# jordanshivers/optical-flow-python

Hardware: AMD Instinct MI355X
Metric: image-pairs/sec at 1920x1080 Classic+NL-fast (+ ms/pyramid-level, AEPE) (higher is better)
Workload: dtype f32; 1 GPU; classic+nl-fast on synth_pair(1080,1920,seed) RGB, 8 pair(s)/GPU/step, 4 in flight; method=classic+nl-fast, height=1080, width=1920, pairs_per_gpu=8, lanes=4, solver=backslash (GPU block-Jacobi PCG surrogate), parallelism=pairs sharded 1/GPU x 1, RCCL gather

## Files before the change

### include/optflow.h

```cpp
#ifndef OPTFLOW_H
#define OPTFLOW_H

#include <stdint.h>

#ifdef __cplusplus
extern "C" {
#endif

#define OF_ABI_VERSION 3

#define OF_OK 0
#define OF_EINVAL (-1)
#define OF_EHIP (-2)
#define OF_ENOMEM (-3)
#define OF_ENOTSUP (-4)
#define OF_ERCCL (-5)

enum of_method { OF_METHOD_HS = 0, OF_METHOD_BA = 1, OF_METHOD_CLASSIC_NL = 2, OF_METHOD_ALT_BA = 3 };

enum of_interp { OF_INTERP_CUBIC = 0 ,
                 OF_INTERP_BICUBIC = 1 ,
                 OF_INTERP_BILINEAR = 2  };

enum of_solver { OF_SOLVER_BACKSLASH = 0, OF_SOLVER_PCG = 1, OF_SOLVER_SOR = 2 };
// ... 83 lines not shown
  double total_ms;
  double preprocess_ms;
} of_stats;

typedef struct of_ctx of_ctx;

int of_abi_version(void);
int of_device_count(int *count);
int of_ctx_create(int device, of_ctx **out);
int of_ctx_destroy(of_ctx *ctx);
const char *of_last_error(of_ctx *ctx);
int of_synchronize(of_ctx *ctx);
int of_set_profiling(of_ctx *ctx, int enable);
#define OF_OPT_SOR_PIPELINE 1
#define OF_OPT_FUSED_WARP 3
int of_set_option(of_ctx *ctx, int option, int value);
#define OF_OPT_SOR_FALLBACKS 2
#define OF_OPT_DEVICE_BYTES 4
#define OF_OPT_RCCL_NRANKS 5
int of_get_option(of_ctx *ctx, int option, int64_t *value);
enum of_event { OF_EV_STAGE = 0, OF_EV_LEVEL = 1, OF_EV_ITER = 2, OF_EV_STAGE_END = 3 };
#define OF_PROGRESS_ITER 1
#define OF_PROGRESS_FLOW 2
typedef struct of_progress {
  int32_t event;
  int32_t stage;
  int32_t level;
  int32_t h, w;
  int32_t iter, lin;
  int32_t pad_;
// ... 103 lines not shown
```

### optical-flow-python_amd/csrc/api.hip

```cpp
extern "C" {

int of_abi_version(void) { return OF_ABI_VERSION; }

int of_device_count(int *count) {
  int n = 0;
  if (hipGetDeviceCount(&n) != hipSuccess) n = 0;
  if (count) *count = n;
  return OF_OK;
}

int of_ctx_create(int device, of_ctx **out) {
  if (!out) return OF_EINVAL;
  *out = nullptr;
  int n = 0;
  if (hipGetDeviceCount(&n) != hipSuccess || device < 0 || device >= n) {
    g_err = "no HIP device";
    return OF_EHIP;
  }
  of_ctx *c = new of_ctx();
  c->device = device;
  try {
    HIPCHK(hipSetDevice(device));
    create_stream(&c->stream);
    HIPCHK(hipMalloc(&c->d_state, sizeof(PcgState)));
// ... 77 lines not shown
  if ((c)->pool) {                                                                   \
    (c)->err = "a pair stream is open on this context (of_pairs_close first)";       \
    return OF_EINVAL;                                                                \
  }

int of_set_option(of_ctx *c, int option, int value) {
  if (!c) return OF_EINVAL;
  REFUSE_WHILE_POOL(c)
  switch (option) {
    case OF_OPT_SOR_PIPELINE:
      c->opt_sor_pipe = value < 0 ? 0 : (value > 2 ? 2 : value);
      return OF_OK;
    case OF_OPT_FUSED_WARP:
      c->opt_fused_warp = value ? 1 : 0;
      return OF_OK;
    default:
      c->err = "unknown option";
      return OF_EINVAL;
  }
}

int of_set_progress(of_ctx *c, of_progress_fn fn, void *user, int flags) {
  if (!c) return OF_EINVAL;
  if (c->pool) pool_set_progress(c->pool, fn);
  else c->prog_fn = fn;
  c->prog_user = user;
  c->prog_flags = flags;
  return OF_OK;
}

int of_get_option(of_ctx *c, int option, int64_t *value) {
  if (!c || !value) return OF_EINVAL;
  switch (option) {
    case OF_OPT_SOR_PIPELINE:
      *value = c->opt_sor_pipe;
      return OF_OK;
    case OF_OPT_FUSED_WARP:
      *value = c->opt_fused_warp;
      return OF_OK;
    case OF_OPT_SOR_FALLBACKS: {
      int64_t n = c->sor_fallbacks;
      for (of_ctx *l : c->lanes) n += l->sor_fallbacks;
      *value = n;
      return OF_OK;
    }
    case OF_OPT_DEVICE_BYTES: {
      auto held = [](const of_ctx *x) {
        return (int64_t)(x->arena.reserved() + x->sor_ring_cap + x->gather_cap);
      };
      int64_t n = held(c);
      for (of_ctx *l : c->lanes) n += held(l);
      *value = n;
      return OF_OK;
// ... 367 lines not shown
  download_f2(c, xx, x);
  HIPCHK(hipStreamSynchronize(c->stream));
  if (iters) *iters = r.iters;
  if (rel_residual) *rel_residual = r.rel;
  API_END(c)
}
int of_detect_occlusion(of_ctx *c, const float *uv, const float *images, int H, int W, int nc, float *occ) {
  API_BEGIN(c)
  REQUIRE(uv && images && occ && nc >= 1, OF_EINVAL, "bad arguments");
  F2 f = upload_f2(c, uv, H, W), z = new_f2(c, H, W), u1 = new_f2(c, H, W);
  fill_f2(c, z, 0.0f);
  Img im = upload_new_img(c, images, H, W, 2 * nc);
  Img o = new_img(c, H, W, 1);
  Grid2 g = grid2(H, W);
  launch(c, "update_occ", k_update_occ, g.grid, g.block, 0, (const float2 *)f.p, (const float2 *)z.p, 0, u1.p,
         (const float *)im.p, (const float *)im.plane(nc), nc, o.p, H, W, f.P, im.ps());
  download_img(c, o, occ);
  HIPCHK(hipStreamSynchronize(c->stream));
  API_END(c)
}

int of_weighted_median(of_ctx *c, const float *uv, const float *guide, int gc, const float *occ, int H, int W,
                       int area_hsz, double sigma_i, float *out) {
  API_BEGIN(c)
  REQUIRE(uv && guide && occ && out && gc >= 1, OF_EINVAL, "bad arguments");
  F2 f = upload_f2(c, uv, H, W), o = new_f2(c, H, W);
  Img g = upload_new_img(c, guide, H, W, gc), oc = upload_new_img(c, occ, H, W, 1);
  wmf(c, f, g, oc.p, o, area_hsz, sigma_i);
  download_f2(c, o, out);
  HIPCHK(hipStreamSynchronize(c->stream));
  API_END(c)
// ... 78 lines not shown
```

### optical-flow-python_amd/csrc/batch.hip

```cpp
namespace {

void ensure_lanes(of_ctx *c, int n) {
  const int want = std::max(n, OF_LANES_MIN - 1);
  while ((int)c->lanes.size() < want) {
    of_ctx *l = nullptr;
    const int rc = of_ctx_create(c->device, &l);
    REQUIRE(rc == OF_OK, rc, "lane context: " + g_err);
    c->lanes.push_back(l);
  }
  if (!c->gstream) create_stream(&c->gstream);
}

of_ctx *lane_ctx(of_ctx *c, int li) { return li ? c->lanes[li - 1] : c; }

void configure_lane(of_ctx *parent, of_ctx *lane, int prof, bool token_on) {
  if (lane != parent) {
    lane->prof = prof;
    lane->epoch = parent->epoch;
  }
  lane->opt_sor_pipe = parent->opt_sor_pipe;
  lane->opt_fused_warp = parent->opt_fused_warp;
  lane->big = token_on && OF_BIG_PX > 0 ? &parent->big_own : nullptr;
  lane->big_px = OF_BIG_PX;
}

void merge_lane_prof(of_ctx *c, int lanes) {
  c->big = nullptr;
  for (int li = 1; li < lanes; ++li) {
    of_ctx *l = c->lanes[li - 1];
    for (auto &kv : l->ktimes) {
      KTime &d = c->ktimes[kv.first];
      d.ms += kv.second.ms;
      d.px += kv.second.px;
      d.n += kv.second.n;
    }
    l->ktimes.clear();
    c->tl.insert(c->tl.end(), l->tl.begin(), l->tl.end());
    l->tl.clear();
// ... 661 lines not shown
```

### optical-flow-python_amd/csrc/host_core.h

```cpp
namespace {

struct OfError {
  int code;
  std::string msg;
};

#define HIPCHK(x)                                                                                    \
  do {                                                                                               \
    hipError_t e_ = (x);                                                                             \
    if (e_ != hipSuccess) throw OfError{OF_EHIP, std::string(#x) + ": " + hipGetErrorString(e_)}; \
  } while (0)
#define REQUIRE(cond, code, msg) \
  do {                           \
    if (!(cond)) throw OfError{code, msg}; \
  } while (0)

#ifndef OF_TOKEN_SLOTS
#define OF_TOKEN_SLOTS 2
#endif
struct Token {
  std::mutex m;
  std::condition_variable cv;
  int free = OF_TOKEN_SLOTS;
  void lock() {
// ... 49 lines not shown
    size_t n = 0;
    for (const auto &c : chunks) n += c.cap;
    return n;
  }
};

struct Img {
  float *p = nullptr;
  int H = 0, W = 0, P = 0, C = 0;
  size_t ps() const { return (size_t)H * P; }
  float *plane(int c) const { return p + (size_t)c * ps(); }
};
struct F2 {
  float2 *p = nullptr;
  int H = 0, W = 0, P = 0;
};

struct ProfRec {
  const char *name;
  hipEvent_t e0, e1;
  double px;
};
struct KTime {
  double ms = 0, px = 0;
  int64_t n = 0;
};

struct Slot {
  void *rgb1 = nullptr, *rgb2 = nullptr;
  float *uv = nullptr;
// ... 123 lines not shown
    const char *name;
    double px, t0, t1;
  };
  std::vector<TlRec> tl;
  hipEvent_t epoch = nullptr;
  bool own_epoch = false;
  std::map<int64_t, int> iter_hints;
  double cur_px = 0;
  std::vector<Slot> slots;
  HostStage *hs = nullptr;
  PairPool *pool = nullptr;
  std::vector<of_ctx *> lanes;
  Token big_own;
  Token *big = nullptr;
  double big_px = 0;
  ncclComm_t comm = nullptr;
  int nranks = 1, rank = 0;
};

namespace {

hipEvent_t next_event(std::vector<hipEvent_t> &pool, size_t &used) {
  if (used == pool.size()) {
    hipEvent_t e;
    HIPCHK(hipEventCreate(&e));
    pool.push_back(e);
  }
  return pool[used++];
}
hipEvent_t pool_event(of_ctx *c) { return next_event(c->ev_pool, c->ev_used); }
// ... 92 lines not shown
```

### optical-flow-python_amd/csrc/host_flow.hip

```cpp
namespace {

OpArgs op_args(const of_params *P, double alpha, double lambda2) {
  OpArgs o;
  memset(&o, 0, sizeof(o));
  o.qd = to_penf(P->qua_data);
  o.rd = to_penf(P->rho_data);
  for (int k = 0; k < 2; ++k) {
    o.qsu[k] = to_penf(P->qua_spatial_u[k]);
    o.qsv[k] = to_penf(P->qua_spatial_v[k]);
    o.rsu[k] = to_penf(P->rho_spatial_u[k]);
    o.rsv[k] = to_penf(P->rho_spatial_v[k]);
  }
  o.rc = to_penf(P->rho_couple);
  o.use_q = alpha > 0.0;
  o.use_r = alpha < 1.0;
  o.aq_s = (float)((o.use_r ? alpha : 1.0) * P->lambda_q);
  o.ar_s = (float)((o.use_q ? 1.0 - alpha : 1.0) * P->lambda_);
  o.aq_d = (float)(o.use_r ? alpha : 1.0);
  o.ar_d = (float)(o.use_q ? 1.0 - alpha : 1.0);
  o.lambda2 = (float)lambda2;
  o.f64 = P->method == OF_METHOD_ALT_BA;
  o.aq_s_d = (o.use_r ? alpha : 1.0) * P->lambda_q;
  o.ar_s_d = (o.use_q ? 1.0 - alpha : 1.0) * P->lambda_;
  o.aq_d_d = o.use_r ? alpha : 1.0;
// ... 67 lines not shown
    if (one) { OF_BY_PM(m, k_warp_operator, 2, 1, ) } else { OF_BY_PM(m, k_warp_operator, 2, 3, ) }
  }
}

struct LevelIn {
  Img im;
  Img guide;
};

struct BigPhase {
  of_ctx *c;
  bool held = false;
  BigPhase(of_ctx *c_, double px) : c(c_) {
    if (c->big && px >= c->big_px) {
      c->big->lock();
      held = true;
    }
  }
  ~BigPhase() {
    if (held) {
      hipStreamSynchronize(c->stream);
      c->big->unlock();
    }
  }
};

SolveResult solve_tok(of_ctx *c, const of_params *P, const Img &coef, const F2 &b, const F2 &x) {
  BigPhase bp(c, (double)b.H * b.W);
  return solve(c, P, coef, b, x);
}

struct ProgressOff {
  of_ctx *c;
  of_progress_fn fn;
  explicit ProgressOff(of_ctx *c_) : c(c_), fn(c_->prog_fn) { c->prog_fn = nullptr; }
  ~ProgressOff() { c->prog_fn = fn; }
// ... 70 lines not shown
  c->cur_px = (double)H * W;
  const double blend = P->method == OF_METHOD_BA ? P->blend : 0.5;
  LevelDeriv D = level_deriv(c, L.im, nc, P->interp, P->deriv_filter, blend);
  Img It = new_img(c, H, W, nc), Ix = new_img(c, H, W, nc), Iy = new_img(c, H, W, nc);
  Img coef = new_img(c, H, W, 7);
  Img occ = new_img(c, H, W, 1);
  F2 rhs = new_f2(c, H, W), x = new_f2(c, H, W), uv1 = new_f2(c, H, W), uv2 = new_f2(c, H, W);
  F2 duv = new_f2(c, H, W);
  OpArgs o = op_args(P, alpha, 0.0);
  Grid2 g = grid2(H, W);
  const bool nl = P->method == OF_METHOD_CLASSIC_NL;
  const bool gen = P->filters.general;
  GenLevel GL;
  if (gen) GL = gen_level(c, P, H, W);
  const bool fuse = !gen && max_linear == 1 && can_fuse_warp_op(c, o, nc);
  for (int it = 0; it < P->max_iters; ++it) {
    if (!fuse) partial_deriv(c, D, P->interp, uv, It, Ix, Iy);
    for (int jl = 0; jl < max_linear; ++jl) {
      if (gen) {
        gen_flow_operator(c, P, o, uv, jl ? &duv : nullptr, It, Ix, Iy, nullptr, GL, rhs);
        note_solve(c, st, gen_solve_logged(c, P, GL, rhs, x));
      } else if (fuse) {
        warp_operator(c, D, P->interp, o, uv, coef, rhs);
        note_solve(c, st, solve_tok(c, P, coef, rhs, x));
      } else {
        flow_operator(c, o, uv, jl ? &duv : nullptr, It, Ix, Iy, nullptr, coef, rhs);
        note_solve(c, st, solve_tok(c, P, coef, rhs, x));
      }
      c->cur_px = (double)H * W;
      prog_iter(c, it, jl, x, jl ? &duv : nullptr, P->limit_update);
      const bool filt = P->median_filter_size != 0;
      launch(c, nl && filt && L.guide.p ? "update_occ" : "update", k_update_occ, g.grid, g.block, 0,
             (const float2 *)uv.p, (const float2 *)x.p, P->limit_update, uv1.p, (const float *)L.im.p,
             (const float *)L.im.plane(nc), nc, (nl && filt && L.guide.p) ? occ.p : (float *)nullptr, H, W, uv.P,
             L.im.ps());
      const bool last = jl + 1 >= max_linear;
      if (last && filt && nl && L.guide.p) {
        wmf(c, uv1, L.guide, occ.p, uv, P->area_hsz, P->sigma_i, (const float2 *)uv.p);
        continue;
      }
      F2 res = uv1;
      if (filt) {
        if (nl && L.guide.p) wmf(c, uv1, L.guide, occ.p, uv2, P->area_hsz, P->sigma_i);
        else median2(c, uv1, uv2, P->median_filter_size);
        res = uv2;
      }
      if (!last)
        launch(c, "sub2", k_sub2, g.grid, g.block, 0, (const float2 *)uv.p, (const float2 *)res.p, duv.p, H, W, uv.P);
      else
        launch(c, "axpy_diff", k_axpy_diff, g.grid, g.block, 0, uv.p, (const float2 *)uv.p, (const float2 *)res.p, H,
// ... 120 lines not shown
    levels = auto_levels(H, W, P->pyramid_spacing);
  P->pyramid_levels = levels;
  REQUIRE(levels <= OF_MAX_LEVELS, OF_EINVAL, "too many pyramid levels");
  FlowPyr F;
  F.levels = levels;
  F.pyr = build_pyramid(c, img, levels, P->pyramid_spacing);
  if (P->method != OF_METHOD_HS) F.gpyr = build_pyramid(c, img, P->gnc_pyramid_levels, P->gnc_pyramid_spacing);
  guide_pyramids(c, P, guide, F);
  return F;
}

void run_schedule(of_ctx *c, of_params *P, const FlowPyr &F, F2 &uv_io, of_stats *st) {
  const int H = uv_io.H, W = uv_io.W, levels = F.levels;
  const std::vector<Img> &pyr = F.pyr, &gpyr = F.gpyr, &cpyr = F.cpyr, &cgpyr = F.cgpyr;
  const bool use_guide = F.use_guide;
  F2 uv = uv_io, uvhat;
  if (P->method == OF_METHOD_ALT_BA) {
    uvhat = new_f2(c, H, W);
    HIPCHK(hipMemcpyAsync(uvhat.p, uv.p, sizeof(float2) * (size_t)H * uv.P, hipMemcpyDeviceToDevice, c->stream));
  }
  const double alpha_orig = P->alpha;
  const int gnc = P->method == OF_METHOD_HS ? 1 : P->gnc_iters;
  std::vector<std::pair<hipEvent_t, hipEvent_t>> lev_ev;
  for (int ig = 0; ig < gnc; ++ig) {
    const int nl = ig == 0 ? levels : P->gnc_pyramid_levels;
    const std::vector<Img> &lv = ig == 0 ? pyr : gpyr;
    c->prog_stage = ig;
    c->prog_level = -1;
    if (c->prog_fn) {
      of_progress e = prog_event(c, OF_EV_STAGE, H, W);
// ... 192 lines not shown
```

### optical-flow-python_amd/csrc/host_image.hip

```cpp
namespace {

Img new_img(of_ctx *c, int H, int W, int C) {
  Img m;
  m.H = H;
  m.W = W;
  m.C = C;
  m.P = of_pitch(W);
  m.p = (float *)c->arena.alloc(sizeof(float) * m.ps() * (C > 0 ? C : 1));
  return m;
}
F2 new_f2(of_ctx *c, int H, int W) {
  F2 f;
  f.H = H;
  f.W = W;
  f.P = of_pitch(W);
  f.p = (float2 *)c->arena.alloc(sizeof(float2) * (size_t)H * f.P);
  return f;
}
Img view(const Img &m, int c0, int n) {
  Img v = m;
  v.p = m.plane(c0);
  v.C = n;
  return v;
}
// ... 173 lines not shown
  Grid2 g = grid2(in.H, in.W);
  const float th = (float)theta, delta = (float)(1.0 / (4.0 * theta));
  const dim3 rg((in.W + ROF_TW - 1) / ROF_TW, (in.H + ROF_TH - 1) / ROF_TH, in.C);
  for (int it = 0; it < iters; it += ROF_K) {
    launch(c, "rof_iters", k_rof_iters, rg, g.block, 0, (const float *)nrm.p, (const float2 *)p0, p1, in.H, in.W,
           nrm.P, ps, th, delta, std::min(ROF_K, iters - it));
    std::swap(p0, p1);
  }
  Img out = new_img(c, in.H, in.W, in.C);
  launch(c, "rof_final", k_rof_final, gz(g, in.C), g.block, 0, (const float *)nrm.p, (const float2 *)p0, out.p, in.H,
         in.W, nrm.P, ps, th, (float)alp);
  scale_img(c, out, 0.0f, 255.0f, 1);
  return out;
}

struct LevelDeriv {
  Img I1x, I1y, A, B, Cc;
  DerivArgs args;
};

LevelDeriv level_deriv(of_ctx *c, const Img &im, int nc, int interp, const double *filt, double blend) {
  LevelDeriv L;
  Img I1 = view(im, 0, nc), I2 = view(im, nc, nc);
  Taps tx = make_taps(filt, 1, 5), ty = make_taps(filt, 5, 1);
  L.I1x = new_img(c, im.H, im.W, nc);
  L.I1y = new_img(c, im.H, im.W, nc);
  correlate(c, I1, L.I1x, tx);
  correlate(c, I1, L.I1y, ty);
  L.A = new_img(c, im.H, im.W, nc);
  L.B = new_img(c, im.H, im.W, nc);
  L.Cc = new_img(c, im.H, im.W, nc);
  correlate(c, I2, L.A, tx);
  correlate(c, I2, L.B, ty);
  if (interp == OF_INTERP_BICUBIC) {
    correlate(c, L.A, L.Cc, ty);
  } else if (interp == OF_INTERP_CUBIC) {
    BsplTaps bt;
    const double z = std::sqrt(3.0) - 2.0, c0 = -6.0 * z / (1.0 - z * z);
    for (int k = 0; k <= OF_BSPL_K; ++k) bt.h[k] = (float)(c0 * std::pow(z, (double)k));
    Img tmp = new_img(c, im.H, im.W, nc);
    Grid2 g = grid2(im.H, im.W);
    auto pf = [&](const Img &src, const Img &dst) {
      launch(c, "bspline_rows", k_bspline_rows, gz(g, nc), g.block, 0, (const float *)src.p, tmp.p, im.H, im.W, im.P,
             im.ps(), bt);
      launch(c, "bspline_cols", k_bspline_cols, gz(g, nc), g.block, 0, (const float *)tmp.p, dst.p, im.H, im.W, im.P,
             im.ps(), bt);
    };
    pf(L.A, L.A);
    pf(L.B, L.B);
    pf(I2, L.Cc);
  }
  DerivArgs &d = L.args;
  d.I1 = I1.p;
  d.I2 = I2.p;
  d.I1x = L.I1x.p;
  d.I1y = L.I1y.p;
  d.A = L.A.p;
  d.B = L.B.p;
  d.Cc = L.Cc.p;
  d.nc = nc;
  d.blend = (float)blend;
  return L;
}

void partial_deriv(of_ctx *c, const LevelDeriv &L, int interp, const F2 &uv, const Img &It, const Img &Ix,
                   const Img &Iy) {
  Grid2 g = grid2(uv.H, uv.W);
  const size_t ps = It.ps();
  auto go = [&](const char *name, auto k) {
    launch(c, name, k, g.grid, g.block, 0, L.args, (const float2 *)uv.p, uv.H, uv.W, uv.P, ps, It.p, Ix.p, Iy.p);
  };
  if (interp == OF_INTERP_BICUBIC) go("partial_deriv_hermite", k_partial_deriv<1>);
  else if (interp == OF_INTERP_CUBIC) go("partial_deriv_bspline", k_partial_deriv<0>);
  else go("partial_deriv_bilinear", k_partial_deriv<2>);
}

// ... 45 lines not shown
```

### optical-flow-python_amd/csrc/host_solve.hip

```cpp
namespace {

struct SolveResult {
  int iters;
  int done;
  double rel;
  int slot = -1;
  double px = 0;
  const char *name = nullptr;
};

Grid2 pair_grid(int H, int W) {
  Grid2 g;
  g.block = dim3(OF_BX, OF_BY, 1);
  int gx = (W + 2 * OF_BX - 1) / (2 * OF_BX), gy = (H + OF_BY - 1) / OF_BY;
  int cap = std::max(1, PCG_MAX_BLOCKS / gx);
  g.grid = dim3(gx, std::min(gy, cap), 1);
  g.nblocks = g.grid.x * g.grid.y;
  return g;
}

template <typename Enq>
int run_chunked(of_ctx *c, int maxiter, int first, int max_chunk, Enq enqueue_iter) {
  int enq = 0, chunk = first, nchunks = 0;
  while (enq < maxiter) {
// ... 2 lines not shown
    enq += n;
    const int slot = nchunks & 1;
    HIPCHK(hipMemcpyAsync(&c->h_state[slot], c->d_state, sizeof(PcgState), hipMemcpyDeviceToHost, c->stream));
    HIPCHK(hipEventRecord(c->ev_state[slot], c->stream));
    ++nchunks;
    if (nchunks >= 2) {
      HIPCHK(hipEventSynchronize(c->ev_state[slot ^ 1]));
      if (c->h_state[slot ^ 1].done) break;
    }
    chunk = nchunks == 1 ? 4 : std::min(std::max(chunk + chunk / 2, 8), max_chunk);
  }
  return enq;
}

template <typename Enq>
int run_fed(of_ctx *c, volatile CgFlag *f, int nmax, int depth, Enq enqueue_iter) {
  f->done = 0;
  f->iter = 0;
  f->upd = 0;
  f->k = -1;
  std::atomic_thread_fence(std::memory_order_seq_cst);
  int enq = 0;
  while (enq < nmax) {
    if (f->done) break;
    if (enq - f->k <= depth) {
      enqueue_iter(enq++);
      continue;
    }
    const auto t0 = std::chrono::steady_clock::now();
    while (!f->done && enq - f->k > depth) {
      _mm_pause();
      if (std::chrono::steady_clock::now() - t0 > std::chrono::milliseconds(500)) {
        HIPCHK(hipStreamSynchronize(c->stream));
        REQUIRE(f->done || f->k == enq - 1, OF_EHIP, "CG progress flag not visible to the host");
        break;
      }
    }
  }
  return enq;
// ... 121 lines not shown
      gy = (nbands + 3) / 4;
    }
  }
  g->grid_x = nstrips;
  g->grid_y = gy;
  g->rows = R;
  g->bands = nbands;
  g->blocks = nstrips * gy;
  g->strip_cols = sw;
  return g->blocks <= PCG_MAX_BLOCKS ? OF_OK : OF_ENOTSUP;
}

#define CG_UPD_FIRST 16
#define CG_UPD_EVERY 8

void log_resid(of_ctx *c, const Img &coef, const F2 &b, const F2 &x, const F2 *xh, double *out) {
  Grid2 g = grid2(b.H, b.W, PCG_MAX_BLOCKS);
  launch(c, "resid", k_resid_part, g.grid, g.block, 0, (const float *)coef.p, coef.ps(), (const float2 *)b.p,
         (const float2 *)x.p, xh ? (const float2 *)xh->p : nullptr, (const PcgState *)(xh ? c->d_state : nullptr),
         b.H, b.W, b.P, c->d_rpart);
  launch(c, "resid", k_resid_final, dim3(1), dim3(OF_BX, OF_BY), 0, (const double *)c->d_rpart, g.nblocks, out);
}

void finish_backslash(of_ctx *c, const Img &coef, const F2 &b, const F2 &x, const F2 &xh) {
  if (c->slog_idx >= 0) {
    log_resid(c, coef, b, x, &xh, c->d_rlog + 4 * c->slog_idx);
    c->slog_iter = true;
  }
  Grid2 g = grid2(x.H, x.W);
  launch(c, "cg_finalize", k_cg_finalize, g.grid, g.block, 0, x.p, (const float2 *)xh.p, (const PcgState *)c->d_state,
         x.H, x.W, x.P);
}

struct CgSetup {
  bool block = false;
  float poly[8] = {0.f, 0.f, 0.f, 0.f, 0.f, 0.f, 0.f, 0.f};
  int slot = 0;
  double rtol = 0, upd_rel = 0;
  int maxiter = 0;
  F2 xh;
};
CgSetup cg_setup(of_ctx *c, const of_params *P, int H, int W) {
// ... 88 lines not shown
  for (int i = 0; i < 8; ++i) a.poly[i] = s.poly[i];
  a.hflag = c->d_flag + s.slot;
  HIPCHK(hipMemsetAsync(c->d_state, 0, sizeof(PcgState), c->stream));
  auto args_k = [&](int k) {
    PcgArgs ak = a;
    const int cur = k & 1, prev = cur ^ 1;
    ak.r_in = rb[prev].p;
    ak.p_old = pb[prev].p;
    ak.r_out = rb[cur].p;
    ak.p_new = pb[cur].p;
    ak.part_rd = c->d_partials + (size_t)prev * 5 * PCG_MAX_BLOCKS;
    ak.part_wr = c->d_partials + (size_t)cur * 5 * PCG_MAX_BLOCKS;
    return ak;
  };
  volatile CgFlag *hf = c->h_flag + s.slot;
  const int enq = run_fed(c, hf, a.maxiter + 1, 3, [&](int k) {
    if (s.upd_rel > 0 && k >= CG_UPD_FIRST && (k - CG_UPD_FIRST) % CG_UPD_EVERY == 0 && !hf->upd)
      launch(c, "cg_update", k_cg_update, grid, blk, 0, args_k(k), k);
    const bool odd = W & 1;
    auto kern = split ? (k == 0 ? (odd ? k_cgs<true, true> : k_cgs<true, false>)
                                : (odd ? k_cgs<false, true> : k_cgs<false, false>))
                      : (k == 0 ? (odd ? k_cg<true, false, true> : k_cg<true, false, false>)
                                : (odd ? k_cg<false, false, true> : k_cg<false, false, false>));
    launch(c, "pcg_iter", kern, grid, blk, 0, args_k(k), k, R, nbands);
  });
  if (!hf->done) launch(c, "pcg_check", k_pcg_check, dim3(1), blk, 0, args_k(enq), enq);
  return cg_queued(c, s, coef, b, x, "pcg_iter");
}

SolveResult sor_result(const PcgState &st) {
  return {st.iter, st.done, st.xnorm2 > 0 ? std::sqrt(st.rr / st.xnorm2) : 0.0};
}

bool sor_outcome(of_ctx *c, const int *fail, SolveResult *r) {
  HIPCHK(hipMemcpyAsync(&c->h_state[0], c->d_state, sizeof(PcgState), hipMemcpyDeviceToHost, c->stream));
  HIPCHK(hipMemcpyAsync(c->h_norm, fail, sizeof(int), hipMemcpyDeviceToHost, c->stream));
  HIPCHK(hipStreamSynchronize(c->stream));
  if (*(const int *)c->h_norm != 0) return false;
  *r = sor_result(c->h_state[0]);
  return true;
}
// ... 348 lines not shown
```

### optical-flow-python_amd/csrc/kernels.h

```cpp
#pragma once
#include "common.h"

#define OF_BSPL_K 16

struct Taps {
  float w[25];
  int kh, kw;
};

struct BsplTaps {
  float h[OF_BSPL_K + 1];
};

struct OpArgs {
  PenF qd, qsu[2], qsv[2];
  PenF rd, rsu[2], rsv[2];
  PenF rc;
  float aq_s, ar_s;
  float aq_d, ar_d;
  int use_q, use_r;
  float lambda2;
  int f64;
  double aq_s_d, ar_s_d, aq_d_d, ar_d_d, lambda2_d;
};
// ... 15 lines not shown

struct PcgState {
  double rho[2];
  double rr;
  double atol;
  double bnorm;
  float alpha, beta;
  int iter;
  int done;
  int maxiter;
  int upd_k;
  int upd_due;
  int pad_;
  double xnorm2, dnorm2;
};
```

### optical-flow-python_amd/csrc/kernels_flow.hip

```cpp
#include "kernels.h"

__device__ __forceinline__ void hermite(float t, float h[4], float dh[4]) {
  OF_NOCONTRACT
  float t2 = t * t, t3 = t2 * t;
  h[0] = 2.0f * t3 - 3.0f * t2 + 1.0f;
  h[1] = -2.0f * t3 + 3.0f * t2;
  h[2] = t3 - 2.0f * t2 + t;
  h[3] = t3 - t2;
  dh[0] = 6.0f * t2 - 6.0f * t;
  dh[1] = -6.0f * t2 + 6.0f * t;
  dh[2] = 3.0f * t2 - 4.0f * t + 1.0f;
  dh[3] = 3.0f * t2 - 2.0f * t;
}

__device__ __forceinline__ float bspline3(float t) {
  OF_NOCONTRACT
  t = fabsf(t);
  if (t < 1.0f) return 2.0f / 3.0f - t * t + 0.5f * t * t * t;
  if (t < 2.0f) {
    float s = 2.0f - t;
    return s * s * s * (1.0f / 6.0f);
  }
  return 0.0f;
}
// ... 334 lines not shown
      avv += o.lambda2_d * tv;
      bu += o.lambda2_d * tu * (h.x - u0.x);
      bv += o.lambda2_d * tv * (h.y - u0.y);
    }
    coef[k] = (float)eR.x;
    coef[ps + k] = (float)eD.x;
    coef[2 * ps + k] = (float)eR.y;
    coef[3 * ps + k] = (float)eD.y;
    coef[4 * ps + k] = (float)auu;
    coef[5 * ps + k] = (float)(psi * ixy);
    coef[6 * ps + k] = (float)avv;
    rhs[k] = make_float2((float)bu, (float)bv);
  }
}

__device__ __forceinline__ float2 upd(const float2 *uv, const float2 *x, size_t k, int clip) {
  float2 a = uv[k], b = x[k];
  if (clip) { b.x = fminf(fmaxf(b.x, -1.0f), 1.0f); b.y = fminf(fmaxf(b.y, -1.0f), 1.0f); }
  return make_float2(a.x + b.x, a.y + b.y);
}

__global__ void k_update_occ(const float2 *__restrict__ uv, const float2 *__restrict__ x, int clip,
                             float2 *__restrict__ uv1, const float *__restrict__ I1, const float *__restrict__ I2,
                             int nc, float *__restrict__ occ, int H, int W, int P, size_t ps) {
  OF_FOR_PIXELS_XCD(H, W) {
    if (j >= W) continue;
    const size_t k = (size_t)i * P + j;
    const float2 c = upd(uv, x, k, clip);
    uv1[k] = c;
    if (!occ) continue;
    float dudx = j > 0 ? c.x - upd(uv, x, k - 1, clip).x : 0.0f;
    float dvdy = i > 0 ? c.y - upd(uv, x, k - P, clip).y : 0.0f;
    float div = dudx + dvdy;
    float odiv = expf(-div * div * (1.0f / (2.0f * 0.3f * 0.3f)));
    float r = fminf(fmaxf((float)i + c.y, 0.0f), (float)(H - 1));
    float q = fminf(fmaxf((float)j + c.x, 0.0f), (float)(W - 1));
    int i0 = (int)floorf(r), j0 = (int)floorf(q);
    float fr = r - i0, fc = q - j0;
    int i1 = min(i0 + 1, H - 1), j1 = min(j0 + 1, W - 1);
    float it = 0.0f;
    for (int ch = 0; ch < nc; ++ch) {
      const float *b = I2 + ch * ps;
      const float *r0 = b + (size_t)i0 * P, *r1 = b + (size_t)i1 * P;
      float w = (1.0f - fr) * ((1.0f - fc) * r0[j0] + fc * r0[j1]) + fr * ((1.0f - fc) * r1[j0] + fc * r1[j1]);
      it += fabsf(w - I1[ch * ps + k]);
    }
    if (nc > 1) it /= (float)nc;
// ... 34 lines not shown

__global__ void k_fb_check(const float2 *__restrict__ fw, const float2 *__restrict__ bw, int H, int W, int P,
                           double alpha1, double alpha2, uint8_t *__restrict__ st_fw, float *__restrict__ er_fw,
                           uint8_t *__restrict__ st_bw, float *__restrict__ er_bw) {
  OF_FOR_PIXELS_XCD(H, W) {
    if (j >= W) continue;
    fb_check_px(fw, bw, i, j, H, W, P, alpha1, alpha2, st_fw, er_fw);
    if (st_bw) fb_check_px(bw, fw, i, j, H, W, P, alpha1, alpha2, st_bw, er_bw);
  }
}

__global__ void k_add_update(float2 *__restrict__ uv, const float2 *__restrict__ x, int clip, int H, int W, int P) {
  OF_FOR_PIXELS(H, W) {
    if (j >= W) continue;
    const size_t k = (size_t)i * P + j;
    uv[k] = upd(uv, x, k, clip);
  }
}

__global__ void k_axpy_diff(float2 *__restrict__ uv, const float2 *__restrict__ a, const float2 *__restrict__ b, int H,
                            int W, int P) {
  OF_FOR_PIXELS(H, W) {
    if (j >= W) continue;
    const size_t k = (size_t)i * P + j;
    float2 u = uv[k], x = a[k], y = b[k];
    uv[k] = make_float2(u.x + (y.x - x.x), u.y + (y.y - x.y));
  }
}

__global__ void k_sub2(const float2 *__restrict__ a, const float2 *__restrict__ b, float2 *__restrict__ out, int H,
                       int W, int P) {
// ... 536 lines not shown
```

### optical-flow-python_amd/csrc/kernels_img.hip

```cpp
#include "kernels.h"

__global__ void k_mm_init(uint32_t *mm, int n) {
  int t = threadIdx.x;
  if (t < n) { mm[2 * t] = 0xffffffffu; mm[2 * t + 1] = 0u; }
}

__global__ void k_minmax(const float *__restrict__ a, int H, int W, int P, int planes, size_t plane_stride,
                         uint32_t *mm) {
  uint32_t lo = 0xffffffffu, hi = 0u;
  OF_FOR_PIXELS(H, W) {
    if (j < W)
      for (int c = 0; c < planes; ++c) {
        uint32_t o = f2ord(a[c * plane_stride + (size_t)i * P + j]);
        lo = min(lo, o);
        hi = max(hi, o);
      }
  }
  for (int off = 32; off > 0; off >>= 1) {
    lo = min(lo, (uint32_t)__shfl_down((int)lo, off, 64));
    hi = max(hi, (uint32_t)__shfl_down((int)hi, off, 64));
  }
  __shared__ uint32_t s_lo[OF_BY], s_hi[OF_BY];
  if (threadIdx.x == 0) {
    s_lo[threadIdx.y] = lo;
// ... 193 lines not shown
    if (j >= W) continue;
    int cols[KW];
#pragma unroll
    for (int b = 0; b < KW; ++b) cols[b] = refl1(j + b - cw, W);
    float s = 0.0f;
#pragma unroll
    for (int a = 0; a < KH; ++a) {
      const float *row = in + (size_t)refl1(i + a - ch, H) * P;
#pragma unroll
      for (int b = 0; b < KW; ++b) {
        const float w = t.w[a * KW + b];
        if (w != 0.0f) s += w * row[cols[b]];
      }
    }
    out[(size_t)i * P + j] = s;
  }
}

template <typename T>
__global__ void k_resize(const T *__restrict__ in, int H, int W, int P, size_t ps, T *__restrict__ out, int nH, int nW,
                         int nP, size_t nps, float mult) {
  in += blockIdx.z * ps;
  out += blockIdx.z * nps;
  const float sy = (float)H / (float)nH, sx = (float)W / (float)nW;
  const int j = blockIdx.x * OF_BX + threadIdx.x;
  if (j >= nW) return;
  float c = fminf(fmaxf((j + 0.5f) * sx - 0.5f, 0.0f), (float)(W - 1));
  int j0 = (int)floorf(c);
  float fc = c - j0;
  int j1 = min(j0 + 1, W - 1);
// ... 155 lines not shown
```

### optical-flow-python_amd/csrc/kernels_solve.hip

```cpp
#include "kernels.h"

#define PCG_MAX_BLOCKS 512
static_assert(PCG_MAX_BLOCKS % 256 == 0,
              "the CG prologue sums PCG_MAX_BLOCKS / 256 partials per lane of a 256-thread block: a remainder would "
              "be left out");
#define CG_DEG 5

template <bool BLOCK>
__device__ __forceinline__ float2 precond(float a, float c, float d, float2 r) {
  if (BLOCK) {
    const float det = a * d - c * c;
    if (det > 1e-30f * fabsf(a * d)) {
      const float inv = 1.0f / det;
      return make_float2((d * r.x - c * r.y) * inv, (a * r.y - c * r.x) * inv);
    }
  }
  return make_float2(fabsf(a) > 1e-12f ? r.x / a : 0.0f, fabsf(d) > 1e-12f ? r.y / d : 0.0f);
}

template <int NV>
__device__ __forceinline__ void prologue_sum(double (&out)[NV], const double *__restrict__ part, int nb, double *lds) {
  const int tid = threadIdx.x + threadIdx.y * blockDim.x, nt = blockDim.x * blockDim.y;
#pragma unroll
  for (int v = 0; v < NV; ++v) {
// ... 1298 lines not shown
    const int i = e / W, j = e - i * W;
    const size_t kk = (size_t)i * P + j;
    const double2 rv = resid_px(g.coef, g.ps, g.b, g.x, nullptr, i, j, H, W, P);
    const float2 rf = make_float2((float)rv.x, (float)rv.y);
    r[kk] = rf;
    g.xh[kk] = g.x[kk];
    acc[0] += (double)rf.x * rf.x + (double)rf.y * rf.y;
  }
  write_partials<1>(acc, const_cast<double *>(g.part_rd) + 4 * PCG_MAX_BLOCKS, lds);
  if (tid == 0 && bid == 0) {
    g.st->upd_k = k;
    if (g.hflag) __hip_atomic_store(&g.hflag->upd, 1, __ATOMIC_RELAXED, __HIP_MEMORY_SCOPE_SYSTEM);
  }
}

__device__ __forceinline__ bool cg_xlo_live(const PcgState *st) { return st->iter >= st->upd_k; }

__global__ __launch_bounds__(256) void k_cg_finalize(float2 *x, const float2 *__restrict__ xh,
                                                     const PcgState *st, int H, int W, int P) {
  if (!st->upd_k) return;
  const bool lo = cg_xlo_live(st);
  OF_FOR_PIXELS(H, W) {
    if (j >= W) continue;
    const size_t k = (size_t)i * P + j;
    const float2 a = lo ? x[k] : make_float2(0.f, 0.f), h = xh[k];
    x[k] = make_float2((float)((double)a.x + (double)h.x), (float)((double)a.y + (double)h.y));
  }
}

#ifndef SOR_D
#define SOR_D 7
#endif
#ifndef SOR_G
#define SOR_G 8
#endif
#define SOR_MAXS (PCG_MAX_BLOCKS / 2)

struct SorArgs {
  const float *coef;
  const float2 *b;
  float2 *x;
// ... 725 lines not shown
```

### optical-flow-python_amd/optical_flow/_abi.py

```python
import ctypes as C

OF_ABI_VERSION = 3

OF_OK, OF_EINVAL, OF_EHIP, OF_ENOMEM, OF_ENOTSUP, OF_ERCCL = 0, -1, -2, -3, -4, -5

METHOD = {"hs": 0, "ba": 1, "classic_nl": 2, "alt_ba": 3}
INTERP = {"cubic": 0, "bi-cubic": 1, "bi-linear": 2}
SOLVER = {"backslash": 0, "pcg": 1, "sor": 2}
PENALTY = {
    "quadratic": 0, "lorentzian": 1, "charbonnier": 2, "generalized_charbonnier": 3,
    "geman_mcclure": 4, "huber": 5, "tukey": 6, "gaussian": 7, "tdist": 8, "tdist_unnorm": 9,
    "const": 100,
}
MAX_LEVELS = 32
OF_OPT_SOR_PIPELINE = 1
OF_OPT_SOR_FALLBACKS = 2
OF_OPT_FUSED_WARP = 3
OF_OPT_DEVICE_BYTES = 4
OF_OPT_RCCL_NRANKS = 5


class OfPenalty(C.Structure):
    _fields_ = [("kind", C.c_int32), ("pad_", C.c_int32), ("p0", C.c_double), ("p1", C.c_double)]


_INT_FIELDS = [
    "method", "solver", "interp", "texture", "fc", "auto_level", "pyramid_levels", "gnc_iters",
    "gnc_pyramid_levels", "max_iters", "max_warping_iters", "max_linear", "pcg_maxiter",
    "sor_max_iters", "limit_update", "median_filter_size", "mf_iter", "use_wmf", "area_hsz",
    "itersLO", "exact_maxiter", "display", "guide_mode", "pad_",
]
_DBL_FIELDS = [
    "lambda_", "lambda_q", "alpha", "pyramid_spacing", "gnc_pyramid_spacing", "pcg_rtol",
# ... 89 lines not shown
```

Baseline: 51.46 pairs/s.

## Fuse level derivative filters, cache derivatives, fold CG finalize, lean solver tail

Adds a single shared-memory kernel that computes all five image-derivative planes per level in one pass, replacing five separate correlate launches. Derivatives are cached per image within a pyramid run, and the CG finalize pass is folded into the update kernel. The feed depth of the iteration loop is reduced near the expected convergence count, and the big-phase token is released early once the solver finishes. All of this sits behind new options that default to on; it adds cache state and token bookkeeping, and a stale cache entry could be returned if buffers are reused.

After: 51.78 pairs/s, median of 5. No clear change (+0.6%).

```diff
diff --git a/include/optflow.h b/include/optflow.h
--- a/include/optflow.h
+++ b/include/optflow.h
@@ -121,6 +121,9 @@
 int of_set_profiling(of_ctx *ctx, int enable);
 #define OF_OPT_SOR_PIPELINE 1
 #define OF_OPT_FUSED_WARP 3
+#define OF_OPT_LEAN_TAIL 6
+#define OF_OPT_BIG_PX 7
+#define OF_OPT_FUSED_DERIV 8
 int of_set_option(of_ctx *ctx, int option, int value);
 #define OF_OPT_SOR_FALLBACKS 2
 #define OF_OPT_DEVICE_BYTES 4
diff --git a/optical-flow-python_amd/csrc/api.hip b/optical-flow-python_amd/csrc/api.hip
--- a/optical-flow-python_amd/csrc/api.hip
+++ b/optical-flow-python_amd/csrc/api.hip
@@ -115,6 +115,15 @@
     case OF_OPT_FUSED_WARP:
       c->opt_fused_warp = value ? 1 : 0;
       return OF_OK;
+    case OF_OPT_LEAN_TAIL:
+      c->opt_lean_tail = value ? 1 : 0;
+      return OF_OK;
+    case OF_OPT_BIG_PX:
+      c->opt_big_px = value < 0 ? 0 : value;
+      return OF_OK;
+    case OF_OPT_FUSED_DERIV:
+      c->opt_fused_deriv = value ? 1 : 0;
+      return OF_OK;
     default:
       c->err = "unknown option";
       return OF_EINVAL;
@@ -138,6 +147,15 @@
       return OF_OK;
     case OF_OPT_FUSED_WARP:
       *value = c->opt_fused_warp;
+      return OF_OK;
+    case OF_OPT_LEAN_TAIL:
+      *value = c->opt_lean_tail;
+      return OF_OK;
+    case OF_OPT_BIG_PX:
+      *value = c->opt_big_px;
+      return OF_OK;
+    case OF_OPT_FUSED_DERIV:
+      *value = c->opt_fused_deriv;
       return OF_OK;
     case OF_OPT_SOR_FALLBACKS: {
       int64_t n = c->sor_fallbacks;
@@ -535,7 +553,8 @@
   Img o = new_img(c, H, W, 1);
   Grid2 g = grid2(H, W);
   launch(c, "update_occ", k_update_occ, g.grid, g.block, 0, (const float2 *)f.p, (const float2 *)z.p, 0, u1.p,
-         (const float *)im.p, (const float *)im.plane(nc), nc, o.p, H, W, f.P, im.ps());
+         (const float *)im.p, (const float *)im.plane(nc), nc, o.p, H, W, f.P, im.ps(),
+         (const float2 *)nullptr, (const PcgState *)nullptr);
   download_img(c, o, occ);
   HIPCHK(hipStreamSynchronize(c->stream));
   API_END(c)
diff --git a/optical-flow-python_amd/csrc/batch.hip b/optical-flow-python_amd/csrc/batch.hip
--- a/optical-flow-python_amd/csrc/batch.hip
+++ b/optical-flow-python_amd/csrc/batch.hip
@@ -20,8 +20,11 @@
   }
   lane->opt_sor_pipe = parent->opt_sor_pipe;
   lane->opt_fused_warp = parent->opt_fused_warp;
+  lane->opt_lean_tail = parent->opt_lean_tail;
+  lane->opt_fused_deriv = parent->opt_fused_deriv;
   lane->big = token_on && OF_BIG_PX > 0 ? &parent->big_own : nullptr;
-  lane->big_px = OF_BIG_PX;
+  lane->big_px = parent->opt_big_px > 0 ? (double)parent->opt_big_px : OF_BIG_PX;
+  lane->big_held = false;
 }
 
 void merge_lane_prof(of_ctx *c, int lanes) {
diff --git a/optical-flow-python_amd/csrc/host_core.h b/optical-flow-python_amd/csrc/host_core.h
--- a/optical-flow-python_amd/csrc/host_core.h
+++ b/optical-flow-python_amd/csrc/host_core.h
@@ -87,6 +87,17 @@
 struct F2 {
   float2 *p = nullptr;
   int H = 0, W = 0, P = 0;
+};
+
+struct LevelDeriv {
+  Img I1x, I1y, A, B, Cc;
+  DerivArgs args;
+};
+struct DerivCacheEntry {
+  const float *im;
+  int H, W, nc, interp;
+  double blend;
+  LevelDeriv L;
 };
 
 struct ProfRec {
@@ -240,6 +251,14 @@
   Token big_own;
   Token *big = nullptr;
   double big_px = 0;
+  bool big_held = false;
+  int opt_lean_tail = 1;
+  int opt_fused_deriv = 1;
+  std::vector<DerivCacheEntry> deriv_cache;
+  bool deriv_cache_on = false;
+  int opt_big_px = 0;
+  bool fold_finalize = false;
+  F2 fin_xh;
   ncclComm_t comm = nullptr;
   int nranks = 1, rank = 0;
 };
diff --git a/optical-flow-python_amd/csrc/host_flow.hip b/optical-flow-python_amd/csrc/host_flow.hip
--- a/optical-flow-python_amd/csrc/host_flow.hip
+++ b/optical-flow-python_amd/csrc/host_flow.hip
@@ -105,12 +105,13 @@
   BigPhase(of_ctx *c_, double px) : c(c_) {
     if (c->big && px >= c->big_px) {
       c->big->lock();
-      held = true;
+      held = c->big_held = true;
     }
   }
   ~BigPhase() {
-    if (held) {
+    if (held && c->big_held) {
       hipStreamSynchronize(c->stream);
+      c->big_held = false;
       c->big->unlock();
     }
   }
@@ -211,26 +212,34 @@
   GenLevel GL;
   if (gen) GL = gen_level(c, P, H, W);
   const bool fuse = !gen && max_linear == 1 && can_fuse_warp_op(c, o, nc);
+  const bool fold = c->opt_lean_tail && !gen && max_linear == 1 && P->solver == OF_SOLVER_BACKSLASH &&
+                    !(c->prog_fn && (c->prog_flags & OF_PROGRESS_ITER));
+  struct FoldOff {
+    of_ctx *c;
+    ~FoldOff() { c->fold_finalize = false; }
+  } fold_off{c};
   for (int it = 0; it < P->max_iters; ++it) {
     if (!fuse) partial_deriv(c, D, P->interp, uv, It, Ix, Iy);
     for (int jl = 0; jl < max_linear; ++jl) {
       if (gen) {
         gen_flow_operator(c, P, o, uv, jl ? &duv : nullptr, It, Ix, Iy, nullptr, GL, rhs);
         note_solve(c, st, gen_solve_logged(c, P, GL, rhs, x));
-      } else if (fuse) {
-        warp_operator(c, D, P->interp, o, uv, coef, rhs);
+      } else {
+        if (fuse) warp_operator(c, D, P->interp, o, uv, coef, rhs);
+        else flow_operator(c, o, uv, jl ? &duv : nullptr, It, Ix, Iy, nullptr, coef, rhs);
+        c->fold_finalize = fold;
+        c->fin_xh = F2();
         note_solve(c, st, solve_tok(c, P, coef, rhs, x));
-      } else {
-        flow_operator(c, o, uv, jl ? &duv : nullptr, It, Ix, Iy, nullptr, coef, rhs);
-        note_solve(c, st, solve_tok(c, P, coef, rhs, x));
-      }
+        c->fold_finalize = false;
+      }
+      const float2 *fin_xh = fold && !gen ? (const float2 *)c->fin_xh.p : nullptr;
       c->cur_px = (double)H * W;
       prog_iter(c, it, jl, x, jl ? &duv : nullptr, P->limit_update);
       const bool filt = P->median_filter_size != 0;
       launch(c, nl && filt && L.guide.p ? "update_occ" : "update", k_update_occ, g.grid, g.block, 0,
              (const float2 *)uv.p, (const float2 *)x.p, P->limit_update, uv1.p, (const float *)L.im.p,
              (const float *)L.im.plane(nc), nc, (nl && filt && L.guide.p) ? occ.p : (float *)nullptr, H, W, uv.P,
-             L.im.ps());
+             L.im.ps(), fin_xh, (const PcgState *)c->d_state);
       const bool last = jl + 1 >= max_linear;
       if (last && filt && nl && L.guide.p) {
         wmf(c, uv1, L.guide, occ.p, uv, P->area_hsz, P->sigma_i, (const float2 *)uv.p);
@@ -381,6 +390,17 @@
   const int H = uv_io.H, W = uv_io.W, levels = F.levels;
   const std::vector<Img> &pyr = F.pyr, &gpyr = F.gpyr, &cpyr = F.cpyr, &cgpyr = F.cgpyr;
   const bool use_guide = F.use_guide;
+  struct DerivCache {
+    of_ctx *c;
+    explicit DerivCache(of_ctx *c_) : c(c_) {
+      c->deriv_cache.clear();
+      c->deriv_cache_on = true;
+    }
+    ~DerivCache() {
+      c->deriv_cache.clear();
+      c->deriv_cache_on = false;
+    }
+  } deriv_cache(c);
   F2 uv = uv_io, uvhat;
   if (P->method == OF_METHOD_ALT_BA) {
     uvhat = new_f2(c, H, W);
diff --git a/optical-flow-python_amd/csrc/host_image.hip b/optical-flow-python_amd/csrc/host_image.hip
--- a/optical-flow-python_amd/csrc/host_image.hip
+++ b/optical-flow-python_amd/csrc/host_image.hip
@@ -211,25 +211,34 @@
   return out;
 }
 
-struct LevelDeriv {
-  Img I1x, I1y, A, B, Cc;
-  DerivArgs args;
-};
-
 LevelDeriv level_deriv(of_ctx *c, const Img &im, int nc, int interp, const double *filt, double blend) {
+  const bool keep = c->opt_fused_deriv && c->deriv_cache_on;
+  if (keep)
+    for (const DerivCacheEntry &e : c->deriv_cache)
+      if (e.im == im.p && e.H == im.H && e.W == im.W && e.nc == nc && e.interp == interp && e.blend == blend)
+        return e.L;
   LevelDeriv L;
   Img I1 = view(im, 0, nc), I2 = view(im, nc, nc);
   Taps tx = make_taps(filt, 1, 5), ty = make_taps(filt, 5, 1);
   L.I1x = new_img(c, im.H, im.W, nc);
   L.I1y = new_img(c, im.H, im.W, nc);
-  correlate(c, I1, L.I1x, tx);
-  correlate(c, I1, L.I1y, ty);
   L.A = new_img(c, im.H, im.W, nc);
   L.B = new_img(c, im.H, im.W, nc);
   L.Cc = new_img(c, im.H, im.W, nc);
-  correlate(c, I2, L.A, tx);
-  correlate(c, I2, L.B, ty);
-  if (interp == OF_INTERP_BICUBIC) {
+  const bool one_pass = c->opt_fused_deriv && interp == OF_INTERP_BICUBIC && im.H > 2 && im.W > 2;
+  if (one_pass) {
+    DerivTaps dt;
+    for (int a = 0; a < 5; ++a) dt.w[a] = (float)filt[a];
+    const dim3 grid((im.W + LD_TW - 1) / LD_TW, (im.H + LD_TH - 1) / LD_TH, nc);
+    launch(c, "correlate", k_level_deriv, grid, dim3(OF_BX, OF_BY), 0, (const float *)I1.p, (const float *)I2.p,
+           L.I1x.p, L.I1y.p, L.A.p, L.B.p, L.Cc.p, im.H, im.W, im.P, im.ps(), dt);
+  } else {
+    correlate(c, I1, L.I1x, tx);
+    correlate(c, I1, L.I1y, ty);
+    correlate(c, I2, L.A, tx);
+    correlate(c, I2, L.B, ty);
+  }
+  if (interp == OF_INTERP_BICUBIC && !one_pass) {
     correlate(c, L.A, L.Cc, ty);
   } else if (interp == OF_INTERP_CUBIC) {
     BsplTaps bt;
@@ -257,6 +266,7 @@
   d.Cc = L.Cc.p;
   d.nc = nc;
   d.blend = (float)blend;
+  if (keep) c->deriv_cache.push_back({im.p, im.H, im.W, nc, interp, blend, L});
   return L;
 }
 
diff --git a/optical-flow-python_amd/csrc/host_solve.hip b/optical-flow-python_amd/csrc/host_solve.hip
--- a/optical-flow-python_amd/csrc/host_solve.hip
+++ b/optical-flow-python_amd/csrc/host_solve.hip
@@ -40,7 +40,7 @@
 }
 
 template <typename Enq>
-int run_fed(of_ctx *c, volatile CgFlag *f, int nmax, int depth, Enq enqueue_iter) {
+int run_fed(of_ctx *c, volatile CgFlag *f, int nmax, int depth, int near, int depth_near, Enq enqueue_iter) {
   f->done = 0;
   f->iter = 0;
   f->upd = 0;
@@ -49,6 +49,7 @@
   int enq = 0;
   while (enq < nmax) {
     if (f->done) break;
+    if (enq >= near) depth = depth_near;
     if (enq - f->k <= depth) {
       enqueue_iter(enq++);
       continue;
@@ -200,6 +201,16 @@
 #define CG_UPD_FIRST 16
 #define CG_UPD_EVERY 8
 
+#ifndef CG_FEED_DEPTH
+#define CG_FEED_DEPTH 3
+#endif
+#ifndef CG_FEED_DEPTH_NEAR
+#define CG_FEED_DEPTH_NEAR 1
+#endif
+#ifndef CG_FEED_NEAR
+#define CG_FEED_NEAR 3
+#endif
+
 void log_resid(of_ctx *c, const Img &coef, const F2 &b, const F2 &x, const F2 *xh, double *out) {
   Grid2 g = grid2(b.H, b.W, PCG_MAX_BLOCKS);
   launch(c, "resid", k_resid_part, g.grid, g.block, 0, (const float *)coef.p, coef.ps(), (const float2 *)b.p,
@@ -212,6 +223,9 @@
   if (c->slog_idx >= 0) {
     log_resid(c, coef, b, x, &xh, c->d_rlog + 4 * c->slog_idx);
     c->slog_iter = true;
+  } else if (c->fold_finalize) {
+    c->fin_xh = xh;
+    return;
   }
   Grid2 g = grid2(x.H, x.W);
   launch(c, "cg_finalize", k_cg_finalize, g.grid, g.block, 0, x.p, (const float2 *)xh.p, (const PcgState *)c->d_state,
@@ -330,7 +344,9 @@
     return ak;
   };
   volatile CgFlag *hf = c->h_flag + s.slot;
-  const int enq = run_fed(c, hf, a.maxiter + 1, 3, [&](int k) {
+  int &hint = iter_hint(c, H, W, split ? OF_SOLVER_BACKSLASH : OF_SOLVER_PCG);
+  const int near = c->opt_lean_tail && hint > 0 ? std::max(0, hint + 2 - CG_FEED_NEAR) : a.maxiter + 1;
+  const int enq = run_fed(c, hf, a.maxiter + 1, CG_FEED_DEPTH, near, CG_FEED_DEPTH_NEAR, [&](int k) {
     if (s.upd_rel > 0 && k >= CG_UPD_FIRST && (k - CG_UPD_FIRST) % CG_UPD_EVERY == 0 && !hf->upd)
       launch(c, "cg_update", k_cg_update, grid, blk, 0, args_k(k), k);
     const bool odd = W & 1;
@@ -340,7 +356,15 @@
                                 : (odd ? k_cg<false, false, true> : k_cg<false, false, false>));
     launch(c, "pcg_iter", kern, grid, blk, 0, args_k(k), k, R, nbands);
   });
-  if (!hf->done) launch(c, "pcg_check", k_pcg_check, dim3(1), blk, 0, args_k(enq), enq);
+  if (!hf->done) {
+    launch(c, "pcg_check", k_pcg_check, dim3(1), blk, 0, args_k(enq), enq);
+  } else {
+    hint = hf->iter;
+    if (c->opt_lean_tail && c->big_held) {
+      c->big_held = false;
+      c->big->unlock();
+    }
+  }
   return cg_queued(c, s, coef, b, x, "pcg_iter");
 }
 
diff --git a/optical-flow-python_amd/csrc/kernels.h b/optical-flow-python_amd/csrc/kernels.h
--- a/optical-flow-python_amd/csrc/kernels.h
+++ b/optical-flow-python_amd/csrc/kernels.h
@@ -6,6 +6,10 @@
 struct Taps {
   float w[25];
   int kh, kw;
+};
+
+struct DerivTaps {
+  float w[5];
 };
 
 struct BsplTaps {
@@ -53,3 +57,11 @@
   int pad_;
   double xnorm2, dnorm2;
 };
+
+__device__ __forceinline__ bool cg_xlo_live(const PcgState *st) { return st->iter >= st->upd_k; }
+
+__device__ __forceinline__ float2 cg_final_x(const float2 *x, const float2 *xh, size_t k, bool fin, bool lo) {
+  if (!fin) return x[k];
+  const float2 a = lo ? x[k] : make_float2(0.f, 0.f), h = xh[k];
+  return make_float2((float)((double)a.x + (double)h.x), (float)((double)a.y + (double)h.y));
+}
diff --git a/optical-flow-python_amd/csrc/kernels_flow.hip b/optical-flow-python_amd/csrc/kernels_flow.hip
--- a/optical-flow-python_amd/csrc/kernels_flow.hip
+++ b/optical-flow-python_amd/csrc/kernels_flow.hip
@@ -372,23 +372,26 @@
   }
 }
 
-__device__ __forceinline__ float2 upd(const float2 *uv, const float2 *x, size_t k, int clip) {
-  float2 a = uv[k], b = x[k];
+__device__ __forceinline__ float2 upd(const float2 *uv, const float2 *x, const float2 *xh, bool fin, bool lo, size_t k,
+                                      int clip) {
+  float2 a = uv[k], b = cg_final_x(x, xh, k, fin, lo);
   if (clip) { b.x = fminf(fmaxf(b.x, -1.0f), 1.0f); b.y = fminf(fmaxf(b.y, -1.0f), 1.0f); }
   return make_float2(a.x + b.x, a.y + b.y);
 }
 
 __global__ void k_update_occ(const float2 *__restrict__ uv, const float2 *__restrict__ x, int clip,
                              float2 *__restrict__ uv1, const float *__restrict__ I1, const float *__restrict__ I2,
-                             int nc, float *__restrict__ occ, int H, int W, int P, size_t ps) {
+                             int nc, float *__restrict__ occ, int H, int W, int P, size_t ps,
+                             const float2 *__restrict__ xh, const PcgState *__restrict__ st) {
+  const bool fin = xh && st->upd_k, lo = fin && cg_xlo_live(st);
   OF_FOR_PIXELS_XCD(H, W) {
     if (j >= W) continue;
     const size_t k = (size_t)i * P + j;
-    const float2 c = upd(uv, x, k, clip);
+    const float2 c = upd(uv, x, xh, fin, lo, k, clip);
     uv1[k] = c;
     if (!occ) continue;
-    float dudx = j > 0 ? c.x - upd(uv, x, k - 1, clip).x : 0.0f;
-    float dvdy = i > 0 ? c.y - upd(uv, x, k - P, clip).y : 0.0f;
+    float dudx = j > 0 ? c.x - upd(uv, x, xh, fin, lo, k - 1, clip).x : 0.0f;
+    float dvdy = i > 0 ? c.y - upd(uv, x, xh, fin, lo, k - P, clip).y : 0.0f;
     float div = dudx + dvdy;
     float odiv = expf(-div * div * (1.0f / (2.0f * 0.3f * 0.3f)));
     float r = fminf(fmaxf((float)i + c.y, 0.0f), (float)(H - 1));
@@ -453,7 +456,7 @@
   OF_FOR_PIXELS(H, W) {
     if (j >= W) continue;
     const size_t k = (size_t)i * P + j;
-    uv[k] = upd(uv, x, k, clip);
+    uv[k] = upd(uv, x, nullptr, false, false, k, clip);
   }
 }
 
diff --git a/optical-flow-python_amd/csrc/kernels_img.hip b/optical-flow-python_amd/csrc/kernels_img.hip
--- a/optical-flow-python_amd/csrc/kernels_img.hip
+++ b/optical-flow-python_amd/csrc/kernels_img.hip
@@ -231,6 +231,56 @@
       }
     }
     out[(size_t)i * P + j] = s;
+  }
+}
+
+#define LD_TW OF_BX
+#define LD_TH 16
+__device__ __forceinline__ float corr5(const DerivTaps &t, float v0, float v1, float v2, float v3, float v4) {
+  float s = 0.0f;
+  if (t.w[0] != 0.0f) s += t.w[0] * v0;
+  if (t.w[1] != 0.0f) s += t.w[1] * v1;
+  if (t.w[2] != 0.0f) s += t.w[2] * v2;
+  if (t.w[3] != 0.0f) s += t.w[3] * v3;
+  if (t.w[4] != 0.0f) s += t.w[4] * v4;
+  return s;
+}
+__global__ __launch_bounds__(OF_BX *OF_BY) void k_level_deriv(const float *__restrict__ I1, const float *__restrict__ I2,
+                                                             float *__restrict__ I1x, float *__restrict__ I1y,
+                                                             float *__restrict__ I2x, float *__restrict__ I2y,
+                                                             float *__restrict__ I2xy, int H, int W, int P, size_t ps,
+                                                             DerivTaps t) {
+  constexpr int RH = LD_TH + 4, RW = LD_TW + 4;
+  __shared__ float s1[RH][RW], s2[RH][RW], sx[RH][LD_TW];
+  const size_t zo = blockIdx.z * ps;
+  I1 += zo;
+  I2 += zo;
+  const int i0 = blockIdx.y * LD_TH, j0 = blockIdx.x * LD_TW;
+  const int tid = threadIdx.x + threadIdx.y * OF_BX;
+  for (int e = tid; e < RH * RW; e += OF_BX * OF_BY) {
+    const int r = e / RW, q = e - r * RW;
+    const int gi = min(max(refl1(i0 - 2 + r, H), 0), H - 1), gj = min(max(refl1(j0 - 2 + q, W), 0), W - 1);
+    const size_t k = (size_t)gi * P + gj;
+    s1[r][q] = I1[k];
+    s2[r][q] = I2[k];
+  }
+  __syncthreads();
+  for (int e = tid; e < RH * LD_TW; e += OF_BX * OF_BY) {
+    const int r = e / LD_TW, q = e - r * LD_TW;
+    sx[r][q] = corr5(t, s2[r][q], s2[r][q + 1], s2[r][q + 2], s2[r][q + 3], s2[r][q + 4]);
+  }
+  __syncthreads();
+  const int q = threadIdx.x, j = j0 + q;
+  if (j >= W) return;
+  for (int r = threadIdx.y; r < LD_TH; r += OF_BY) {
+    const int i = i0 + r;
+    if (i >= H) break;
+    const size_t k = zo + (size_t)i * P + j;
+    I1x[k] = corr5(t, s1[r + 2][q], s1[r + 2][q + 1], s1[r + 2][q + 2], s1[r + 2][q + 3], s1[r + 2][q + 4]);
+    I1y[k] = corr5(t, s1[r][q + 2], s1[r + 1][q + 2], s1[r + 2][q + 2], s1[r + 3][q + 2], s1[r + 4][q + 2]);
+    I2x[k] = sx[r + 2][q];
+    I2y[k] = corr5(t, s2[r][q + 2], s2[r + 1][q + 2], s2[r + 2][q + 2], s2[r + 3][q + 2], s2[r + 4][q + 2]);
+    I2xy[k] = corr5(t, sx[r][q], sx[r + 1][q], sx[r + 2][q], sx[r + 3][q], sx[r + 4][q]);
   }
 }
 
diff --git a/optical-flow-python_amd/csrc/kernels_solve.hip b/optical-flow-python_amd/csrc/kernels_solve.hip
--- a/optical-flow-python_amd/csrc/kernels_solve.hip
+++ b/optical-flow-python_amd/csrc/kernels_solve.hip
@@ -1336,8 +1336,6 @@
   }
 }
 
-__device__ __forceinline__ bool cg_xlo_live(const PcgState *st) { return st->iter >= st->upd_k; }
-
 __global__ __launch_bounds__(256) void k_cg_finalize(float2 *x, const float2 *__restrict__ xh,
                                                      const PcgState *st, int H, int W, int P) {
   if (!st->upd_k) return;
@@ -1345,8 +1343,7 @@
   OF_FOR_PIXELS(H, W) {
     if (j >= W) continue;
     const size_t k = (size_t)i * P + j;
-    const float2 a = lo ? x[k] : make_float2(0.f, 0.f), h = xh[k];
-    x[k] = make_float2((float)((double)a.x + (double)h.x), (float)((double)a.y + (double)h.y));
+    x[k] = cg_final_x(x, xh, k, true, lo);
   }
 }
 
diff --git a/optical-flow-python_amd/optical_flow/_abi.py b/optical-flow-python_amd/optical_flow/_abi.py
--- a/optical-flow-python_amd/optical_flow/_abi.py
+++ b/optical-flow-python_amd/optical_flow/_abi.py
@@ -17,6 +17,9 @@
 OF_OPT_SOR_FALLBACKS = 2
 OF_OPT_FUSED_WARP = 3
 OF_OPT_DEVICE_BYTES = 4
+OF_OPT_LEAN_TAIL = 6
+OF_OPT_BIG_PX = 7
+OF_OPT_FUSED_DERIV = 8
 OF_OPT_RCCL_NRANKS = 5
 
 
```
